# iKrishneel/fcn_object_detector

Measured on AMD Instinct MI355X. Metric: frames/sec forward 448x448 @1 GPU; train imgs/sec @1/2/4/8 GPUs, higher is better.
Workload: dtype f32

## Files before the change

### fcn_object_detector_amd/csrc/train.hip

```cpp
#include <math.h>

#include <type_traits>

#include "common.h"

using namespace fcn;

typedef float f32x16 __attribute__((ext_vector_type(16)));
typedef float v4f __attribute__((ext_vector_type(4)));

namespace {

typedef const void __attribute__((address_space(1))) * gvoid_cptr;
typedef void __attribute__((address_space(3))) * lds_ptr;
typedef float __attribute__((address_space(1))) * gf_ptr;

template <int N>
__device__ __forceinline__ void wait_vmcnt() { asm volatile("s_waitcnt vmcnt(%0)" ::"n"(N) : "memory"); }

struct WgradP {
    const float* x;
    const float* dy;
    float* dw_part;
    float* db_part;
// ... 883 lines not shown
                                                                int H, int W, int C, int dx_cstride, int dx_coffset, int k, int stride, int pad,
                                                                int OH, int OW, int dy_cstride, int dy_coffset, int accumulate,
                                                                const float* __restrict__ relu_y, int ry_cstride, int ry_coffset, int cgroups) {
    const int cg = (int)blockIdx.x % cgroups, tx = (int)blockIdx.x / cgroups;
    const int c = cg * 32 + ((int)threadIdx.x & 7) * 4;
    const int pp = (int)threadIdx.x >> 3;
    const int iy = (int)blockIdx.y * 8 + (pp >> 3), ix = tx * 8 + (pp & 7), n = (int)blockIdx.z;
    if (c >= C || iy >= H || ix >= W) return;
    const int oy_lo = max(0, (iy + pad - k + stride) / stride), oy_hi = min(OH - 1, (iy + pad) / stride);
    const int ox_lo = max(0, (ix + pad - k + stride) / stride), ox_hi = min(OW - 1, (ix + pad) / stride);
    const int me = iy * W + ix;
    v4f g = {0.f, 0.f, 0.f, 0.f};
    for (int oy = oy_lo; oy <= oy_hi; ++oy)
        for (int ox = ox_lo; ox <= ox_hi; ++ox) {
            const size_t o = ((size_t)(n * OH + oy) * OW + ox);
            const int4 id = *reinterpret_cast<const int4*>(idx + o * C + c);
            const v4f d = *reinterpret_cast<const v4f*>(dy + o * dy_cstride + dy_coffset + c);
            g[0] += id.x == me ? d[0] : 0.f;
            g[1] += id.y == me ? d[1] : 0.f;
            g[2] += id.z == me ? d[2] : 0.f;
            g[3] += id.w == me ? d[3] : 0.f;
        }
    const size_t pix = (size_t)(n * H + iy) * W + ix;
    v4f* dst = reinterpret_cast<v4f*>(dx + pix * dx_cstride + dx_coffset + c);
    if (accumulate) g += *dst;
    if (relu_y) {
        const v4f y = *reinterpret_cast<const v4f*>(relu_y + pix * ry_cstride + ry_coffset + c);
#pragma unroll
        for (int e = 0; e < 4; ++e) g[e] = y[e] > 0.f ? g[e] : 0.f;
    }
    *dst = g;
}

__global__ __launch_bounds__(256) void lrn_bwd_kernel(const float* __restrict__ x, const float* __restrict__ y, const float* __restrict__ scale,
                                                      const float* __restrict__ dy, float* __restrict__ dx, long long pixels, int C,
                                                      int x_cstride, int y_cstride, int local_size, float ratio2ab, float beta, int accumulate) {
    const long long total = pixels * C;
    const int pre = (local_size - 1) / 2;
    for (long long t = (long long)blockIdx.x * blockDim.x + threadIdx.x; t < total; t += (long long)gridDim.x * blockDim.x) {
        const int c = (int)(t % C);
        const long long pix = t / C;
        const float* yp = y + (size_t)pix * y_cstride;
        const float* dyp = dy + (size_t)pix * y_cstride;
        const float* sp = scale + (size_t)pix * C;
        float acc = 0.f;
        for (int j = c - (local_size - 1 - pre); j <= c + pre; ++j)
            if (j >= 0 && j < C) acc += dyp[j] * yp[j] / sp[j];
        const float g = dyp[c] * powf(sp[c], -beta) - ratio2ab * x[(size_t)pix * x_cstride + c] * acc;
        float* d = dx + (size_t)pix * x_cstride + c;
        *d = accumulate ? *d + g : g;
    }
}

__global__ __launch_bounds__(256) void lrn5_bwd_kernel(const float* __restrict__ x, const float* __restrict__ y, const float* __restrict__ scale,
                                                       const float* __restrict__ dy, float* __restrict__ dx, long long pixels, int C,
                                                       int x_cstride, int y_cstride, float ratio2ab, float beta, int accumulate) {
    const int cg = C / 4;
    const long long total = pixels * cg;
    const v4f zero = {0.f, 0.f, 0.f, 0.f};
    for (long long t = (long long)blockIdx.x * blockDim.x + threadIdx.x; t < total; t += (long long)gridDim.x * blockDim.x) {
        const long long pix = t / cg;
        const int g = (int)(t - pix * cg);
        const float* yp = y + (size_t)pix * y_cstride + g * 4;
        const float* dyp = dy + (size_t)pix * y_cstride + g * 4;
        const float* sp = scale + (size_t)pix * C + g * 4;
        const bool hl = g > 0, hr = g + 1 < cg;
// ... 642 lines not shown
}

int fcn_relu_bwd_f32(const float* dy, const float* y, float* dx, int pixels, int C, int cstride, fcn_stream_t s) {
    FCN_REQUIRE(dy && y && dx && pixels > 0 && C > 0 && cstride >= C, FCN_E_ARG, "relu_bwd: bad args");
    hipStream_t st = as_stream(s);
    if (cstride == C)
        hipLaunchKernelGGL(relu_bwd_kernel, dim3(stream_grid((long long)pixels * C, 256)), dim3(256), 0, st, dy, y, dx, (size_t)pixels * C);
    else
        hipLaunchKernelGGL(relu_bwd_view_kernel, dim3(stream_grid((long long)pixels * C, 256)), dim3(256), 0, st, dy, y, dx, (long long)pixels, C,
                           cstride);
    FCN_LAUNCH_CHECK("relu_bwd");
    return 0;
}

int fcn_sigmoid_bwd_f32(const float* y, const float* dy, float* dx, size_t count, int accumulate, fcn_stream_t s) {
    FCN_REQUIRE(y && dy && dx, FCN_E_ARG, "sigmoid_bwd: null");
    if (!count) return 0;
    hipLaunchKernelGGL(sigmoid_bwd_kernel, dim3(stream_grid((long long)count, 256)), dim3(256), 0, as_stream(s), y, dy, dx, count, accumulate);
    FCN_LAUNCH_CHECK("sigmoid_bwd");
    return 0;
}

int fcn_maxpool_bwd_mask_f32(const float* dy, const int32_t* idx, float* dx, int N, int H, int W, int C, int dx_cstride, int dx_coffset, int k,
                             int stride, int pad, int OH, int OW, int dy_cstride, int dy_coffset, int accumulate, const float* relu_y,
                             int relu_y_cstride, int relu_y_coffset, fcn_stream_t s) {
    FCN_REQUIRE(dy && idx && dx && N > 0 && H > 0 && W > 0 && C > 0 && k > 0 && stride > 0 && OH > 0 && OW > 0, FCN_E_ARG, "maxpool_bwd: bad args");
    FCN_REQUIRE(dx_cstride >= dx_coffset + C && dy_cstride >= dy_coffset + C, FCN_E_ARG, "maxpool_bwd: channel slice out of range");
    FCN_REQUIRE(!relu_y || (relu_y_coffset >= 0 && relu_y_cstride >= relu_y_coffset + C), FCN_E_ARG, "maxpool_bwd: mask slice out of range");
    const bool v4 = C % 4 == 0 && dx_cstride % 4 == 0 && dx_coffset % 4 == 0 && dy_cstride % 4 == 0 && dy_coffset % 4 == 0 &&
                    (long long)N * H * W * (C / 4) < (1ll << 31) && (((uintptr_t)dy | (uintptr_t)idx | (uintptr_t)dx) & 15) == 0 &&
                    (!relu_y || (relu_y_cstride % 4 == 0 && relu_y_coffset % 4 == 0 && ((uintptr_t)relu_y & 15) == 0));
    const int cgroups = (C + 31) / 32;
    const long long gx = (long long)cgroups * ((W + 7) / 8);
    if (v4 && gx < (1ll << 31) && (H + 7) / 8 <= 65535 && N <= 65535)
        hipLaunchKernelGGL(maxpool_bwd_patch_kernel, dim3((unsigned)gx, (H + 7) / 8, N), dim3(512), 0, as_stream(s), dy, idx, dx, H, W, C, dx_cstride,
                           dx_coffset, k, stride, pad, OH, OW, dy_cstride, dy_coffset, accumulate, relu_y, relu_y_cstride, relu_y_coffset, cgroups);
    else if (v4)
        hipLaunchKernelGGL(maxpool_bwd_v4_kernel, dim3(stream_grid((long long)N * H * W * (C / 4), 256)), dim3(256), 0, as_stream(s), dy, idx, dx, N, H,
                           W, C, dx_cstride, dx_coffset, k, stride, pad, OH, OW, dy_cstride, dy_coffset, accumulate, relu_y, relu_y_cstride,
                           relu_y_coffset);
    else
        hipLaunchKernelGGL(maxpool_bwd_kernel, dim3(stream_grid((long long)N * H * W * C, 256)), dim3(256), 0, as_stream(s), dy, idx, dx, N, H, W, C,
                           dx_cstride, dx_coffset, k, stride, pad, OH, OW, dy_cstride, dy_coffset, accumulate, relu_y, relu_y_cstride, relu_y_coffset);
    FCN_LAUNCH_CHECK("maxpool_bwd");
    return 0;
}

int fcn_maxpool_bwd_f32(const float* dy, const int32_t* idx, float* dx, int N, int H, int W, int C, int dx_cstride, int dx_coffset, int k,
                        int stride, int pad, int OH, int OW, int dy_cstride, int dy_coffset, int accumulate, fcn_stream_t s) {
    return fcn_maxpool_bwd_mask_f32(dy, idx, dx, N, H, W, C, dx_cstride, dx_coffset, k, stride, pad, OH, OW, dy_cstride, dy_coffset, accumulate,
                                    nullptr, 0, 0, s);
}

int fcn_deconv_depthwise_bwd_f32(const float* dy, const float* w, float* dx, int N, int H, int W, int C, int dx_cstride, int k, int stride,
                                 int pad, int OH, int OW, int dy_cstride, int dy_coffset, int accumulate, fcn_stream_t s) {
    FCN_REQUIRE(dy && w && dx && N > 0 && H > 0 && W > 0 && C > 0 && k > 0 && stride > 0 && pad >= 0, FCN_E_ARG, "deconv_bwd: bad args");
    FCN_REQUIRE(OH == stride * (H - 1) + k - 2 * pad && OW == stride * (W - 1) + k - 2 * pad, FCN_E_ARG,
                "deconv_bwd: OH/OW do not match s(H-1)+k-2p");
    FCN_REQUIRE(dx_cstride >= C && dy_coffset >= 0 && dy_cstride >= dy_coffset + C, FCN_E_ARG, "deconv_bwd: channel slice out of range");
    hipLaunchKernelGGL(deconv_dw_bwd_kernel, dim3(stream_grid((long long)N * H * W * C, 256)), dim3(256), 0, as_stream(s), dy, w, dx, N, H, W, C,
                       dx_cstride, k, stride, pad, OH, OW, dy_cstride, dy_coffset, accumulate);
    FCN_LAUNCH_CHECK("deconv_depthwise_bwd");
    return 0;
}

size_t fcn_softmax_loss_workspace_bytes(void) { return (size_t)SML_MAX_BLOCKS * 2 * sizeof(double) + 64; }

int fcn_softmax_loss_f32(const float* x, const float* label, float* dx, float* d_loss, int N, int pixels, int C, int x_cstride,
                         int label_cstride, int normalize, int has_ignore, int ignore_label, float weight, void* d_workspace, fcn_stream_t s) {
    FCN_REQUIRE(x && label && d_loss && d_workspace && N > 0 && pixels > 0 && C > 0 && x_cstride >= C && label_cstride >= 1, FCN_E_ARG,
                "softmax_loss: bad args");
    FCN_REQUIRE(((uintptr_t)d_workspace & 7) == 0, FCN_E_ALIGN, "softmax_loss: workspace must be 8-byte aligned");
    hipStream_t st = as_stream(s);
    int blocks = cdiv(pixels, 256);
    if (blocks > SML_MAX_BLOCKS) blocks = SML_MAX_BLOCKS;
    double* partial = reinterpret_cast<double*>(d_workspace);
    float* d_scale = reinterpret_cast<float*>(partial + (size_t)SML_MAX_BLOCKS * 2);
    hipLaunchKernelGGL(softmax_loss_partial_kernel, dim3(blocks), dim3(256), 0, st, x, label, dx, partial, (long long)pixels, C, x_cstride,
                       label_cstride, has_ignore, ignore_label);
    hipLaunchKernelGGL(softmax_loss_final_kernel, dim3(1), dim3(64), 0, st, partial, blocks, d_loss, d_scale, N, normalize, weight);
    if (dx) hipLaunchKernelGGL(scale_view_kernel, dim3(stream_grid((long long)pixels * C, 256)), dim3(256), 0, st, dx, d_scale, (long long)pixels, C,
                               x_cstride);
    FCN_LAUNCH_CHECK("softmax_loss");
    return 0;
// ... 62 lines not shown
```

### fcn_object_detector_amd/lib.py

```python
from __future__ import annotations

import ctypes as C
import os
import threading
from typing import Optional

_HERE = os.path.dirname(os.path.abspath(__file__))
LIB_PATH = os.environ.get("FCN_LIB_PATH") or os.path.join(_HERE, "libfcnhip.so")


class FcnLibraryError(RuntimeError):
    pass


class FcnError(RuntimeError):
    def __init__(self, code: int, msg: str):
        super().__init__("libfcnhip error %d: %s" % (code, msg))
        self.code = code


class ConvDesc(C.Structure):
    _fields_ = [
        ("x", C.c_void_p), ("w", C.c_void_p), ("bias", C.c_void_p), ("y", C.c_void_p), ("y2", C.c_void_p),
        ("N", C.c_int32), ("H", C.c_int32), ("W", C.c_int32), ("Cin", C.c_int32), ("x_cstride", C.c_int32),
# ... 11 lines not shown
class ConvGroup(C.Structure):
    _fields_ = [("d_probs", C.c_void_p), ("n", C.c_int32), ("cfg", C.c_int32), ("total_tiles", C.c_int32)]


class SolverSeg(C.Structure):
    _fields_ = [("offset", C.c_uint64), ("count", C.c_uint64), ("lr_mult", C.c_float), ("decay_mult", C.c_float)]


class LayoutDesc(C.Structure):
    _fields_ = [("src", C.c_void_p), ("dst", C.c_void_p)] + [(k, C.c_int32) for k in ("N", "C", "H", "W", "src_cstride", "src_coffset")]


class PoolDesc(C.Structure):
    _fields_ = [("x", C.c_void_p), ("y", C.c_void_p), ("idx", C.c_void_p)] + [(k, C.c_int32) for k in (
        "N", "H", "W", "C", "x_cstride", "k", "stride", "pad", "OH", "OW", "y_cstride", "y_coffset", "f16")]


class SceneObj(C.Structure):
    _fields_ = [("img", C.c_void_p), ("mask", C.c_void_p)] + [(k, C.c_int32) for k in (
        "src_h", "src_w", "flip", "roi_x", "roi_y", "roi_w", "roi_h", "out_w", "out_h", "cx", "cy", "label1")]


class ColorParams(C.Structure):
    _fields_ = [("sharpen_centre", C.c_float), ("sharpen_off", C.c_float), ("add", C.c_int32 * 3), ("mul", C.c_float * 3),
                ("gray_alpha", C.c_float), ("gray_keep", C.c_float)]


GAUSS_MAX_RADIUS = 15


class FlipSeg(C.Structure):
    _fields_ = [("w_offset", C.c_uint64), ("wt_offset", C.c_uint64), ("Cout", C.c_int32), ("kh", C.c_int32), ("kw", C.c_int32),
                ("Cin", C.c_int32), ("Cin4", C.c_int32), ("Cout4", C.c_int32)]


class DetectParams(C.Structure):
    _fields_ = [
        ("num_classes", C.c_int32), ("gy", C.c_int32), ("gx", C.c_int32), ("cell_w", C.c_int32), ("cell_h", C.c_int32),
        ("cvg_cstride", C.c_int32), ("cvg_coffset", C.c_int32), ("box_cstride", C.c_int32), ("box_coffset", C.c_int32),
        ("prob_thresh", C.c_float), ("group_thresh", C.c_int32), ("eps", C.c_double), ("min_height", C.c_int32),
        ("round_mode", C.c_int32), ("max_out", C.c_int32),
    ]


CONV_RELU, CONV_SIGMOID2, CONV_ACCUM, CONV_OUT_F32, CONV_F16, CONV_OUT_F16, CONV_MASK = 1, 2, 4, 8, 16, 32, 64
CONV_IMAGE_ONES = 128
ELT_PROD, ELT_SUM, ELT_MAX = 0, 1, 2
RECT_ROUND_NEAREST_EVEN, RECT_ROUND_TRUNCATE = 0, 1

_vp, _i, _f, _d, _sz = C.c_void_p, C.c_int, C.c_float, C.c_double, C.c_size_t

PROTOTYPES = {
    "fcn_abi_version": (_i, []),
    "fcn_last_error_string": (C.c_char_p, []),
    "fcn_device_count": (_i, [C.POINTER(_i)]),
    "fcn_init": (_i, [_i]),
    "fcn_device_name": (_i, [C.c_char_p, _i]),
    "fcn_device_sync": (_i, []),
    "fcn_malloc": (_i, [C.POINTER(_vp), _sz]),
    "fcn_free": (_i, [_vp]),
    "fcn_host_malloc": (_i, [C.POINTER(_vp), _sz]),
    "fcn_host_free": (_i, [_vp]),
    "fcn_memset_async": (_i, [_vp, _i, _sz, _vp]),
    "fcn_memcpy_h2d_async": (_i, [_vp, _vp, _sz, _vp]),
    "fcn_memcpy_d2h_async": (_i, [_vp, _vp, _sz, _vp]),
    "fcn_memcpy_d2d_async": (_i, [_vp, _vp, _sz, _vp]),
# ... 54 lines not shown
    "fcn_conv2d_wgrad_workspace_floats_cfg": (_sz, [C.POINTER(ConvDesc), _i, C.POINTER(_i)]),
    "fcn_conv2d_wgrad_cfg_f32": (_i, [C.POINTER(ConvDesc), _vp, _vp, _vp, _i, _vp]),
    "fcn_conv2d_wgrad_group_workspace_floats_cfg": (_sz, [C.POINTER(ConvDesc), _i, _i]),
    "fcn_conv2d_wgrad_group_cfg_f32": (_i, [C.POINTER(ConvDesc), _vp, _vp, _i, _vp, _i, _vp]),
    "fcn_conv_weights_flip_f32": (_i, [_vp, _vp, _i, _i, _i, _i, _i, _i, _vp]),
    "fcn_nchw_f32_to_nhwc_f16": (_i, [_vp, _vp, _i, _i, _i, _i, _i, _i, _f, _vp]),
    "fcn_nhwc_f16_to_nchw_f32": (_i, [_vp, _vp, _i, _i, _i, _i, _i, _i, _vp]),
    "fcn_maxpool_fwd_f16": (_i, [_vp, _vp] + [_i] * 12 + [_vp]),
    "fcn_lrn_fwd_f16": (_i, [_vp, _vp, _i, _i, _i, _i, _i, _f, _f, _f, _vp]),
    "fcn_avepool_fwd_f16": (_i, [_vp, _vp] + [_i] * 12 + [_vp]),
    "fcn_deconv_depthwise_fwd_f16": (_i, [_vp, _vp, _vp, _vp] + [_i] * 13 + [_vp]),
    "fcn_eltwise_fwd_f16": (_i, [_vp, _vp, _vp, _sz, _i, _f, _f, _vp]),
    "fcn_softmax_fwd_f16": (_i, [_vp, _vp, _i, _i, _i, _i, _i, _vp]),
    "fcn_copy_channels_f16": (_i, [_vp, _vp, _i, _i, _i, _i, _i, _i, _vp]),
    "fcn_preprocess_bgr8_batch": (_i, [_vp, _i, _i, _i, _vp, _i, _i, _i, _i, _f, _vp, _vp]),
    "fcn_preprocess_bgr8_rois": (_i, [_vp, _i, _i, _vp, _i, _vp, _i, _i, _i, _i, _f, _vp, _vp]),
    "fcn_preprocess_bgr8_f16": (_i, [_vp, _i, _i, _vp, _i, _i, _i, _f, _vp, _vp]),
    "fcn_compose_scene_bgr8": (_i, [_vp, _i, _i, _i, _i, _i, _i, _vp, _i, _i, _vp, _vp, _i, _i, _vp]),
    "fcn_mask_to_label_f32": (_i, [_vp, _i, _i, _vp, _i, _i, _i, _vp]),
    "fcn_compose_scene_view_bgr8": (_i, [_vp, _i, _i, _i, _i, _i, _i, _vp, _i, _i, _vp, _vp, _i, _i, _i, _i, _i, _i, _vp]),
    "fcn_blur_gauss_bgr8": (_i, [_vp, _vp, _vp, _i, _i, _vp, _i, _vp]),
    "fcn_blur_box_bgr8": (_i, [_vp, _vp, _i, _i, _i, _vp]),
    "fcn_blur_median_bgr8": (_i, [_vp, _vp, _i, _i, _i, _vp]),
    "fcn_color_augment_bgr8": (_i, [_vp, _vp, _i, _i, _vp, _vp]),
    "fcn_softmax_fwd_f32": (_i, [_vp, _vp, _i, _i, _i, _i, _vp]),
    "fcn_softmax_loss_workspace_bytes": (_sz, []),
    "fcn_softmax_loss_f32": (_i, [_vp, _vp, _vp, _vp, _i, _i, _i, _i, _i, _i, _i, _i, _f, _vp, _vp]),
    "fcn_deconv_depthwise_bwd_f32": (_i, [_vp, _vp, _vp] + [_i] * 13 + [_vp]),
    "fcn_conv_weights_flip_batch_f32": (_i, [_vp, _vp, _vp, _i, _vp]),
    "fcn_relu_bwd_f32": (_i, [_vp, _vp, _vp, _i, _i, _i, _vp]),
    "fcn_sigmoid_bwd_f32": (_i, [_vp, _vp, _vp, _sz, _i, _vp]),
    "fcn_maxpool_bwd_f32": (_i, [_vp, _vp, _vp] + [_i] * 14 + [_vp]),
    "fcn_maxpool_bwd_mask_f32": (_i, [_vp, _vp, _vp] + [_i] * 14 + [_vp, _i, _i, _vp]),
    "fcn_lrn_bwd_f32": (_i, [_vp, _vp, _vp, _vp, _vp, _i, _i, _i, _i, _i, _f, _f, _i, _vp]),
    "fcn_dropout_f32": (_i, [_vp, _vp] + [_i] * 8 + [_f, C.c_uint, C.c_uint, _vp]),
    "fcn_stream_wait_event": (_i, [_vp, _vp]),
    "fcn_comm_unique_id": (_i, [C.c_char_p]),
    "fcn_comm_init": (_i, [C.POINTER(_vp), C.c_char_p, _i, _i]),
    "fcn_comm_allreduce_sum_f32": (_i, [_vp, _vp, _sz, _vp]),
    "fcn_comm_destroy": (_i, [_vp]),
    "fcn_loss_f32": (_i, [_i, _vp, _vp, _vp, _vp, _i, _i, _i, _i, _f, _vp]),
    "fcn_sgd_update_f32": (_i, [_vp, _vp, _vp, _vp, _i, _f, _f, _f, _f, _vp]),
    "fcn_adam_update_f32": (_i, [_vp, _vp, _vp, _vp, _vp, _i, _f, _f, _f, _f, _f, _i, _f, _vp]),
}

HW_QUEUES: dict = {}
_lib: Optional[C.CDLL] = None
_lock = threading.Lock()


def load() -> C.CDLL:
    global _lib
    if _lib is not None:
        return _lib
    with _lock:
        if _lib is not None:
            return _lib
        if not os.path.isfile(LIB_PATH):
            raise FcnLibraryError(
                "libfcnhip.so not found at %s — build it with `python -c 'import __graft_entry__ as g; g.build()'` "
                "or `make -C fcn_object_detector_amd/csrc`. There is no CPU fallback." % LIB_PATH)
        global HW_QUEUES
        if "GPU_MAX_HW_QUEUES" in os.environ:
            HW_QUEUES = {"value": os.environ["GPU_MAX_HW_QUEUES"], "set_by": "environment"}
        elif os.environ.get("FCN_SET_HW_QUEUES", "1") != "0":
            os.environ["GPU_MAX_HW_QUEUES"] = "16"
# ... 33 lines not shown
```

### fcn_object_detector_amd/train.py

```python
from __future__ import annotations

import ctypes as C
import os
import math
from typing import Callable, Dict, List, Optional, Sequence, Tuple

import numpy as np

from . import lib as L
from . import proto
from .engine import Blob, DevView, DeviceBuffer, Engine, Op, PinnedArray, _r4
from .netspec import DATA_TYPES, LOSS_TYPES, Layer, NetSpec, kernel_stride_pad

F32 = np.float32


class SolverParams:

    def __init__(self, msg: Optional[proto.Msg] = None, **kw):
        g = (lambda k, d=None: msg.get(k, d)) if msg is not None else (lambda k, d=None: d)
        self.net = g("net", g("train_net"))
        self.base_lr = float(kw.get("base_lr", g("base_lr", 0.01)))
        self.momentum = float(kw.get("momentum", g("momentum", 0.0)))
        self.momentum2 = float(kw.get("momentum2", g("momentum2", 0.999)))
# ... 184 lines not shown

        def emit_dgrads(name: str, items: List[Tuple[L.ConvDesc, float]], targets: List[str]) -> dict:
            rec = dict(name=name, descs=[it[0] for it in items], targets=list(targets), grp=L.ConvGroup())
            rec["op"] = Op("dgrad", name, lambda st, g=rec["grp"]: L.check(lib.fcn_conv2d_fwd_group_f32(C.byref(g), st)), sum(it[1] for it in items))
            ops.append(rec["op"])
            dgrad_records.append(rec)
            return rec

        def finish_dgrads() -> None:
            for x, rop in relu_ops.items():
                w = writers.get(x, [])
                rec = w[-1] if w else None
                if not isinstance(rec, dict) or rop not in ops:
                    continue
                if "pool" in rec:
                    if rec["pool"] == x:
                        rec["mask"] = (B[x].buf.ptr, B[x].cstride, B[x].coffset)
                        ops.remove(rop)
                    continue
                d = rec["descs"][rec["targets"].index(x)]
                act = B[x]
                d.y2, d.y2_cstride, d.y2_coffset = act.buf.ptr, act.cstride, act.coffset
                d.flags |= L.CONV_MASK
                ops.remove(rop)
            for rec in dgrad_records:
                n_ = len(rec["descs"])
                arr = (L.ConvDesc * n_)(*rec["descs"])
                gws = DeviceBuffer(int(lib.fcn_conv2d_group_workspace_bytes(n_)), zero=False)
                cfg = self._tuned_cfg("dgrad:" + rec["name"], arr, n_, gws) if self.autotune else -1
                L.call("fcn_conv2d_group_prepare", arr, n_, gws.ptr, cfg, C.byref(rec["grp"]))
                self._keep.extend([arr, gws, rec["grp"]])
                self._group_workspaces.append(gws)
                rec["op"].name = "%s [cfg%d %dwg]" % (rec["name"], rec["grp"].cfg, rec["grp"].total_tiles)

        def wgrad_item(l: Layer, gtop: Blob):
            xb, yb = B[l.bottoms[0]], B[l.tops[0]]
            k, s, pad = kernel_stride_pad(l.sub("convolution_param"))
            n, cin, h, w = xb.shape
            _, cout, oh, ow = yb.shape
            if gtop.coffset % 4 or gtop.cstride % 4:
                raise NotImplementedError("gradient view of %s is not 16-byte aligned" % l.tops[0])
            d = L.ConvDesc()
            d.x, d.y = xb.ptr, gtop.buf.ptr
            d.N, d.H, d.W, d.Cin, d.x_cstride = n, h, w, _r4(cin), xb.cstride
            d.Cout, d.kh, d.kw, d.pad, d.stride, d.OH, d.OW = cout, k, k, pad, s, oh, ow
            d.y_cstride, d.y_coffset = gtop.cstride, gtop.coffset
            self._keep.append(d)
            dw = self._grad_view(l.name, 0)
            db = self._grad_view(l.name, 1) if len(self.params_dev[l.name]) > 1 else None
            return d, dw, db, 2.0 * n * cout * oh * ow * cin * k * k

        def emit_wgrads(layers_: List[Layer], gtops: List[Blob]) -> None:
            nonlocal ws_floats
            todo = [(l_, g_) for l_, g_ in zip(layers_, gtops) if self._learns(l_) and l_.name not in wgrad_done]
            for base in range(0, len(todo), 4):
                chunk = todo[base:base + 4]
                its = [wgrad_item(l_, g_) for l_, g_ in chunk]
                names = [l_.name for l_, _ in chunk]
                sel = {"cfg": -1}
                cfgs = [-1] + (list(range(int(lib.fcn_conv2d_wgrad_num_configs()))) if self.autotune else [])
                if len(its) == 1:
                    d, dw, db, fl = its[0]
                    ws_floats = max([ws_floats] + [int(lib.fcn_conv2d_wgrad_workspace_floats_cfg(C.byref(d), c, None)) for c in cfgs])
                    op = Op("wgrad", names[0], lambda st, d=d, dw=dw, db=db, sel=sel: L.check(lib.fcn_conv2d_wgrad_cfg_f32(
                        C.byref(d), dw.ptr, db.ptr if db else None, self._ws.ptr, sel["cfg"], st)), fl)
                else:
# ... 113 lines not shown
                for bn in l.bottoms:
                    gb = G.get(bn)
                    if gb is None:
                        continue
                    if state(gb) == "full":
                        if gtop.coffset or gb.coffset or gb.cstride != gtop.cstride:
                            raise NotImplementedError("Eltwise SUM backward accumulating into a channel slice")
                        ops.append(Op("eltwise_bwd", l.name + ":" + bn, lambda st, a=gtop, b=gb: L.check(lib.fcn_eltwise_fwd_f32(
                            a.ptr, b.ptr, b.ptr, a.pixels * a.cstride, L.ELT_SUM, 1.0, 1.0, st))))
                    else:
                        ops.append(Op("eltwise_bwd", l.name + ":" + bn, lambda st, a=gtop, b=gb: L.check(lib.fcn_copy_channels_f32(
                            a.buf.ptr, b.buf.ptr, a.pixels, a.channels, a.cstride, a.coffset, b.cstride, b.coffset, st))))
                    mark(gb)
                continue
            gbot = G.get(l.bottoms[0]) if l.bottoms else None
            if gbot is None:
                continue
            acc = 1 if state(gbot) == "full" else 0
            pool_writer = None
            if t == "Pooling":
                pp = l.sub("pooling_param")
                if str(pp.get("pool", "MAX")) != "MAX":
                    raise NotImplementedError("backward of AVE pooling (%s)" % l.name)
                xb, yb = B[l.bottoms[0]], B[l.tops[0]]
                n, c, h, w = xb.shape
                _, _, oh, ow = yb.shape
                k, s, pad = kernel_stride_pad(pp)
                idx = self.aux_dev[l.name]
                prec = dict(pool=l.bottoms[0], mask=(None, 0, 0))
                ops.append(Op("maxpool_bwd", l.name, lambda st, a=gtop, b=gbot, idx=idx, g=(n, h, w, c), kk=(k, s, pad, oh, ow), acc=acc, r=prec:
                              L.check(lib.fcn_maxpool_bwd_mask_f32(a.buf.ptr, idx.ptr, b.buf.ptr, g[0], g[1], g[2], g[3], b.cstride, b.coffset,
                                                                   kk[0], kk[1], kk[2], kk[3], kk[4], a.cstride, a.coffset, acc, r["mask"][0],
                                                                   r["mask"][1], r["mask"][2], st))))
                pool_writer = prec
            elif t == "LRN":
                xb, yb = B[l.bottoms[0]], B[l.tops[0]]
                p = l.sub("lrn_param")
                ls, al, be = int(p.get("local_size", 5)), float(p.get("alpha", 1.0)), float(p.get("beta", 0.75))
                sc = self.aux_dev[l.name]
                if gtop.coffset or gbot.coffset or xb.coffset or yb.coffset:
                    raise NotImplementedError("LRN backward on channel slices")
                ops.append(Op("lrn_bwd", l.name, lambda st, x=xb, y=yb, sc=sc, a=gtop, b=gbot, q=(ls, al, be), acc=acc: L.check(
                    lib.fcn_lrn_bwd_f32(x.ptr, y.ptr, sc.ptr, a.ptr, b.ptr, x.pixels, x.channels, x.cstride, y.cstride, q[0], q[1], q[2], acc, st))))
            elif t == "Dropout":
                if acc:
                    raise NotImplementedError("dropout backward into an already written gradient")
                ratio = float(l.sub("dropout_param").get("dropout_ratio", 0.5))
                n, c, h, w = B[l.bottoms[0]].shape
                ops.append(Op("dropout_bwd", l.name, lambda st, a=gtop, b=gbot, g=(n, c, h, w), r=ratio: L.check(lib.fcn_dropout_f32(
                    a.buf.ptr, b.buf.ptr, g[0], g[1], g[2], g[3], a.cstride, a.coffset, b.cstride, b.coffset, r, self.dropout_seed,
                    self.dropout_index_offset, st))))
            elif t == "Eltwise":
                p = l.sub("eltwise_param")
                opname = str(p.get("operation", "SUM"))
                if opname != "PROD" or len(l.bottoms) != 2:
                    raise NotImplementedError("backward of Eltwise %s" % l.name)
                if l.bottoms[1] in self.need_grad:
                    raise NotImplementedError("Eltwise PROD backward w.r.t. both bottoms (%s)" % l.name)
                if acc:
                    raise NotImplementedError("Eltwise backward into an already written gradient")
                other = B[l.bottoms[1]]
                count = gtop.pixels * gtop.cstride
                if gtop.coffset or gbot.coffset or other.coffset or other.cstride != gtop.cstride:
                    raise NotImplementedError("Eltwise backward on channel slices")
                ops.append(Op("eltwise_bwd", l.name, lambda st, a=gtop, o=other, b=gbot, n=count: L.check(lib.fcn_eltwise_fwd_f32(
                    a.ptr, o.ptr, b.ptr, n, L.ELT_PROD, 1.0, 1.0, st))))
            elif t == "Deconvolution":
                if any(m != 0.0 for m in l.lr_mult) or not l.lr_mult:
                    raise NotImplementedError("learnable Deconvolution %s (the reference freezes its bilinear upsampling, lr_mult 0)" % l.name)
                p = l.sub("convolution_param")
                k, s, pad = kernel_stride_pad(p)
                xb, yb = B[l.bottoms[0]], B[l.tops[0]]
                n, c, h, w = xb.shape
                _, _, oh, ow = yb.shape
                wdev = self.params_dev[l.name][0].ptr
                ops.append(Op("deconv_bwd", l.name, lambda st, a=gtop, b=gbot, g=(n, h, w, c, k, s, pad, oh, ow), acc=acc, wdev=wdev: L.check(
                    lib.fcn_deconv_depthwise_bwd_f32(a.buf.ptr, wdev, b.ptr, g[0], g[1], g[2], g[3], b.cstride, g[4], g[5], g[6], g[7], g[8],
                                                     a.cstride, a.coffset, acc, st))))
            elif t == "Sigmoid":
                yb = B[l.tops[0]]
                ops.append(Op("sigmoid_bwd", l.name, lambda st, y=yb, a=gtop, b=gbot, acc=acc: L.check(
                    lib.fcn_sigmoid_bwd_f32(y.ptr, a.ptr, b.ptr, y.pixels * y.cstride, acc, st))))
            elif t == "ReLU":
                yb = B[l.tops[0]]
                ops.append(Op("relu_bwd", l.name, lambda st, y=yb, a=gtop, b=gbot: L.check(lib.fcn_relu_bwd_f32(
                    a.ptr, y.ptr, b.ptr, y.pixels, y.channels, y.cstride, st))))
            elif t == "Power":
                continue
            else:
                raise NotImplementedError("backward of layer type %s (%s)" % (t, l.name))
            mark(gbot, pool_writer)
        finish_dgrads()
        self._ws = DeviceBuffer(ws_floats * 4, zero=False)
        self.bwd_ops = ops
        if self.autotune:
            self._tune_wgrads()
        self._plan_buckets()

    def _tune_wgrads(self) -> None:
        lib = L.load()
        ncfg = int(lib.fcn_conv2d_wgrad_num_configs())
        cache = self._load_tune_cache()
        e0, e1 = C.c_void_p(), C.c_void_p()
        L.call("fcn_event_create", C.byref(e0))
        L.call("fcn_event_create", C.byref(e1))
        dirty = False
        for op in self.bwd_ops:
            if op.kind != "wgrad":
                continue
            key = self._tune_key("wgrad:" + "+".join(op.layers))
            if self._tune_from is not None and key in self._tune_from._chosen_cfgs:
                op.sel["cfg"] = self._chosen_cfgs[key] = self._tune_from._chosen_cfgs[key]
                continue
            if cache is not None and key in cache and 0 <= int(cache[key]) < ncfg:
                op.sel["cfg"] = self._chosen_cfgs[key] = int(cache[key])
                continue
            best, best_ms = -1, 1e30
            timed = []
            for cfg in range(ncfg):
                op.sel["cfg"] = cfg
                for _ in range(2):
                    op.run(self.stream)
                L.call("fcn_event_record", e0, self.stream)
                for _ in range(5):
                    op.run(self.stream)
# ... 206 lines not shown
                    L.call("fcn_event_record", e0, self.comm_stream)
                for b in self.buckets:
                    self.comm.all_reduce_sum(scratch.ptr + 4 * b["offset"], b["count"], self.comm_stream)
            L.call("fcn_event_record", e1, self.comm_stream)
            L.call("fcn_event_sync", e1)
            ms = C.c_float()
            L.call("fcn_event_elapsed_ms", e0, e1, C.byref(ms))
            L.call("fcn_event_destroy", e0)
            L.call("fcn_event_destroy", e1)
            scratch.free()
        nbytes = 4 * sum(b["count"] for b in self.buckets)
        us = ms.value * 1e3 / reps
        g = self.comm.world
        return {"allreduce_us": us, "bytes": nbytes, "buckets": len(self.buckets),
                "bus_GBps": (2.0 * (g - 1) / g * nbytes / (us * 1e-6) / 1e9) if us > 0 else 0.0}

    def step_end(self) -> Dict[str, float]:
        with self.lock:
            L.call("fcn_event_sync", self._step_done)
            for b in self.blobs.values():
                b.host_valid = b.is_input
            for nm in self._in_flight:
                self.blobs[nm].host_valid = False
            out = {k: float(v[0]) for k, v in self.loss_host.items()}
            out["total_loss"] = float(sum(self.loss_blobs[k] * out[k] for k in self.loss_blobs))
            out.setdefault("loss", out["total_loss"])
            self.iter += 1
            return out

    DYNAMIC_KINDS = ("dropout", "dropout_bwd")

    def _wgrad_stream(self) -> Optional[int]:
        import os
        if os.environ.get("FCN_WGRAD_STREAM", "1") == "0":
            return None
        if getattr(self, "_side_stream", None) is None:
            sp, ev = C.c_void_p(), C.c_void_p()
            L.call("fcn_stream_create", C.byref(sp))
            L.call("fcn_event_create", C.byref(ev))
            self._side_stream, self._side_done = int(sp.value), ev
        return self._side_stream

    def _step_plan(self) -> List[Tuple[str, object]]:
        if getattr(self, "_plan", None) is not None:
            return self._plan
        import os
        first = not getattr(self, "_warm", False)
        self._warm = True
        use_graph = os.environ.get("FCN_TRAIN_GRAPH", "1") != "0" and os.environ.get("FCN_NO_GRAPH", "0") in ("", "0") and not first
        triggers: Dict[int, List[dict]] = {}
        for b in self.buckets:
            triggers.setdefault(b["after_op"], []).append(b)
        seq: List[Tuple[str, object]] = [("op", op) for op in self.ops]
        for i, op in enumerate(self.bwd_ops):
            seq.append(("op", op))
            if i in triggers:
                seq.append(("reduce", triggers[i]))
        plan: List[Tuple[str, object]] = []
        run: List[Op] = []

        def flush() -> None:
            if not run:
                return
            if use_graph and len(run) > 1:
                L.call("fcn_graph_begin", self.stream)
                try:
                    for op in run:
# ... 137 lines not shown
```

### include/fcnhip.h

```cpp
#ifndef FCNHIP_H_
#define FCNHIP_H_

#include <stddef.h>
#include <stdint.h>

#ifdef __cplusplus
extern "C" {
#endif

#define FCN_ABI_VERSION 1

#define FCN_E_ARG       1
#define FCN_E_ALIGN     2
#define FCN_E_UNSUPPORTED 3
#define FCN_E_STATE     4
#define FCN_E_CAPACITY  5

typedef void* fcn_stream_t;
typedef void* fcn_event_t;
typedef void* fcn_graph_t;
typedef void* fcn_comm_t;

int  fcn_abi_version(void);
const char* fcn_last_error_string(void);
// ... 205 lines not shown
                     uint8_t* pmap, int frame_h, int frame_w, void* d_workspace, int32_t* out, fcn_stream_t s);

int  fcn_gen_targets(const int32_t* rects, const int32_t* labels, const int32_t* rect_offsets, int batch,
                     int num_classes, int gy, int gx, int stride, double iou_thresh,
                     float* foreground, float* bbox, float* size, float* obj, float* cvg_block,
                     fcn_stream_t s);
int  fcn_gen_targets_nhwc(const int32_t* rects, const int32_t* labels, const int32_t* rect_offsets, int batch,
                          int num_classes, int gy, int gx, int stride, double iou_thresh,
                          float* foreground, int fg_cstride, float* bbox, float* size, float* obj, float* cvg_block,
                          int blk_cstride, fcn_stream_t s);

size_t fcn_conv2d_wgrad_workspace_floats(const fcn_conv_desc* h_d, int* h_splits);
int  fcn_conv2d_wgrad_f32(const fcn_conv_desc* h_d, float* dw, float* db, float* d_workspace, fcn_stream_t s);
size_t fcn_conv2d_wgrad_group_workspace_floats(const fcn_conv_desc* h_ds, int n);
int  fcn_conv2d_wgrad_group_f32(const fcn_conv_desc* h_ds, float* const* h_dws, float* const* h_dbs, int n, float* d_workspace,
                                fcn_stream_t s);
int  fcn_conv2d_wgrad_num_configs(void);
int  fcn_conv2d_wgrad_split_config(void);
size_t fcn_conv2d_wgrad_workspace_floats_cfg(const fcn_conv_desc* h_d, int cfg_request, int* h_splits);
int  fcn_conv2d_wgrad_cfg_f32(const fcn_conv_desc* h_d, float* dw, float* db, float* d_workspace, int cfg_request, fcn_stream_t s);
size_t fcn_conv2d_wgrad_group_workspace_floats_cfg(const fcn_conv_desc* h_ds, int n, int cfg_request);
int  fcn_conv2d_wgrad_group_cfg_f32(const fcn_conv_desc* h_ds, float* const* h_dws, float* const* h_dbs, int n, float* d_workspace,
                                    int cfg_request, fcn_stream_t s);
int  fcn_conv_weights_flip_f32(const float* w, float* wt, int Cout, int kh, int kw, int Cin, int Cin4, int Cout4, fcn_stream_t s);
typedef struct fcn_flip_seg { uint64_t w_offset, wt_offset; int32_t Cout, kh, kw, Cin, Cin4, Cout4; } fcn_flip_seg;
int  fcn_conv_weights_flip_batch_f32(const float* w_base, float* wt_base, const fcn_flip_seg* d_segs, int nseg, fcn_stream_t s);
int  fcn_relu_bwd_f32(const float* dy, const float* y, float* dx, int pixels, int C, int cstride, fcn_stream_t s);
int  fcn_sigmoid_bwd_f32(const float* y, const float* dy, float* dx, size_t count, int accumulate, fcn_stream_t s);
int  fcn_maxpool_bwd_f32(const float* dy, const int32_t* idx, float* dx, int N, int H, int W, int C, int dx_cstride, int dx_coffset,
                         int k, int stride, int pad, int OH, int OW, int dy_cstride, int dy_coffset, int accumulate, fcn_stream_t s);
int  fcn_maxpool_bwd_mask_f32(const float* dy, const int32_t* idx, float* dx, int N, int H, int W, int C, int dx_cstride, int dx_coffset,
                              int k, int stride, int pad, int OH, int OW, int dy_cstride, int dy_coffset, int accumulate,
                              const float* relu_y, int relu_y_cstride, int relu_y_coffset, fcn_stream_t s);
int  fcn_lrn_bwd_f32(const float* x, const float* y, const float* scale, const float* dy, float* dx, int pixels, int C,
                     int x_cstride, int y_cstride, int local_size, float alpha, float beta, int accumulate, fcn_stream_t s);
int  fcn_dropout_f32(const float* x, float* y, int N, int C, int H, int W, int x_cstride, int x_coffset, int y_cstride,
                     int y_coffset, float ratio, unsigned seed, unsigned index_offset, fcn_stream_t s);
int  fcn_loss_f32(int kind, const float* a, const float* b, float* da, float* d_loss, int pixels, int C, int cstride, int num,
                  float weight, fcn_stream_t s);
size_t fcn_softmax_loss_workspace_bytes(void);
int  fcn_softmax_loss_f32(const float* x, const float* label, float* dx, float* d_loss, int N, int pixels, int C, int x_cstride,
                          int label_cstride, int normalize, int has_ignore, int ignore_label, float weight, void* d_workspace,
                          fcn_stream_t s);
int  fcn_deconv_depthwise_bwd_f32(const float* dy, const float* w, float* dx, int N, int H, int W, int C, int dx_cstride, int k,
                                  int stride, int pad, int OH, int OW, int dy_cstride, int dy_coffset, int accumulate, fcn_stream_t s);
typedef struct fcn_solver_seg { uint64_t offset, count; float lr_mult, decay_mult; } fcn_solver_seg;
int  fcn_sgd_update_f32(float* w, const float* g, float* hist, const fcn_solver_seg* d_segs, int nseg, float rate, float momentum,
                        float weight_decay, float grad_scale, fcn_stream_t s);
int  fcn_adam_update_f32(float* w, const float* g, float* m, float* v, const fcn_solver_seg* d_segs, int nseg, float rate,
                         float beta1, float beta2, float delta, float weight_decay, int t, float grad_scale, fcn_stream_t s);

int  fcn_comm_unique_id(char* h_id128);
int  fcn_comm_init(fcn_comm_t* comm, const char* h_id128, int world, int rank);
int  fcn_comm_allreduce_sum_f32(fcn_comm_t comm, float* buf, size_t count, fcn_stream_t s);
int  fcn_comm_destroy(fcn_comm_t comm);

#ifdef __cplusplus
}
#endif
#endif
```

Measured before the change: 3551.

## Add LDS-tiled grouped maxpool backward for 3x3 stride-1 pools

Adds a new maxpool backward kernel for 3x3 stride-1 pad-1 pools. It stages a 10x10 halo of dy and argmax indices in LDS per 8x8 tile and 32-channel group, then gathers from shared memory instead of issuing repeated global loads. A grouped launch batches up to four independent pool-backward ops into one kernel, with per-problem parameters read from kernarg, to cut launch count; the training graph builder merges consecutive non-aliasing pool ops. It also makes the side wgrad stream default depend on the reported hardware queue count.

Measured after the change: 3544 (median of 6 runs). About the same (-0.2%).

```diff
diff --git a/fcn_object_detector_amd/csrc/train.hip b/fcn_object_detector_amd/csrc/train.hip
--- a/fcn_object_detector_amd/csrc/train.hip
+++ b/fcn_object_detector_amd/csrc/train.hip
@@ -939,6 +939,99 @@
     *dst = g;
 }
 
+constexpr int kMaxPoolGroup = 4;
+struct PoolBwdP {
+    const float* dy;
+    const int32_t* idx;
+    float* dx;
+    const float* relu_y;
+    int H, W, C, dx_cstride, dx_coffset, dy_cstride, dy_coffset, ry_cstride, ry_coffset, accumulate, cgroups, tiles_x, tiles_y, pad_;
+};
+struct PoolBwdGroupArgs {
+    int n;
+    int blk_end[kMaxPoolGroup];
+    PoolBwdP p[kMaxPoolGroup];
+};
+
+__global__ __launch_bounds__(512) void maxpool_bwd_lds_kernel(const PoolBwdGroupArgs a) {
+    __shared__ v4f s_dy[100 * 8];
+    typedef int v4i __attribute__((ext_vector_type(4)));
+    __shared__ v4i s_id[100 * 8];
+    const int b = blockIdx.x;
+    int pi = 0, begin = 0;
+#pragma unroll
+    for (int i = 0; i < kMaxPoolGroup - 1; ++i) {
+        const bool past = i + 1 < a.n && b >= a.blk_end[i];
+        pi += past ? 1 : 0;
+        begin = past ? a.blk_end[i] : begin;
+    }
+    typedef const PoolBwdGroupArgs __attribute__((address_space(4))) * karg_ptr;
+    karg_ptr ka = (karg_ptr)__builtin_amdgcn_kernarg_segment_ptr();
+    union { PoolBwdP p; unsigned w[sizeof(PoolBwdP) / 4]; } u;
+    const unsigned __attribute__((address_space(4)))* src = (const unsigned __attribute__((address_space(4)))*)&ka->p[pi];
+#pragma unroll
+    for (int i = 0; i < (int)(sizeof(PoolBwdP) / 4); ++i) u.w[i] = src[i];
+    const PoolBwdP& p = u.p;
+    typedef const v4f __attribute__((address_space(1))) * gv4_cptr;
+    typedef const v4i __attribute__((address_space(1))) * gi4_cptr;
+    typedef v4f __attribute__((address_space(1))) * gv4_ptr;
+    int t = b - begin;
+    const int cg = t % p.cgroups;
+    t /= p.cgroups;
+    const int tx = t % p.tiles_x;
+    t /= p.tiles_x;
+    const int ty = t % p.tiles_y, n = t / p.tiles_y;
+    const int q = (int)threadIdx.x & 7, c = cg * 32 + q * 4;
+    const bool c_ok = c < p.C;
+    const v4i none = {-1, -1, -1, -1};
+    const v4f zero = {0.f, 0.f, 0.f, 0.f};
+#pragma unroll
+    for (int r = 0; r < 2; ++r) {
+        const int hp = ((int)threadIdx.x >> 3) + r * 64;
+        if (hp < 100) {
+            const int hy = hp / 10, oy = ty * 8 - 1 + hy, ox = tx * 8 - 1 + (hp - hy * 10);
+            v4i id = none;
+            v4f d = zero;
+            if (c_ok && (unsigned)oy < (unsigned)p.H && (unsigned)ox < (unsigned)p.W) {
+                const size_t o = (size_t)(n * p.H + oy) * p.W + ox;
+                id = *(gi4_cptr)(p.idx + o * p.C + c);
+                d = *(gv4_cptr)(p.dy + o * p.dy_cstride + p.dy_coffset + c);
+            }
+            s_id[hp * 8 + q] = id;
+            s_dy[hp * 8 + q] = d;
+        }
+    }
+    const int pp = (int)threadIdx.x >> 3, ly = pp >> 3, lx = pp & 7;
+    const int iy = ty * 8 + ly, ix = tx * 8 + lx;
+    const bool live = c_ok && iy < p.H && ix < p.W;
+    const size_t pix = (size_t)(n * p.H + iy) * p.W + ix;
+    v4f old = zero, y = zero;
+    if (live && p.accumulate) old = *(gv4_cptr)(p.dx + pix * p.dx_cstride + p.dx_coffset + c);
+    if (live && p.relu_y) y = *(gv4_cptr)(p.relu_y + pix * p.ry_cstride + p.ry_coffset + c);
+    __syncthreads();
+    if (!live) return;
+    const int me = iy * p.W + ix;
+    v4f g = zero;
+#pragma unroll
+    for (int wy = 0; wy < 3; ++wy)
+#pragma unroll
+        for (int wx = 0; wx < 3; ++wx) {
+            const int h = ((ly + wy) * 10 + lx + wx) * 8 + q;
+            const v4i id = s_id[h];
+            const v4f d = s_dy[h];
+            g[0] += id[0] == me ? d[0] : 0.f;
+            g[1] += id[1] == me ? d[1] : 0.f;
+            g[2] += id[2] == me ? d[2] : 0.f;
+            g[3] += id[3] == me ? d[3] : 0.f;
+        }
+    if (p.accumulate) g += old;
+    if (p.relu_y) {
+#pragma unroll
+        for (int e = 0; e < 4; ++e) g[e] = y[e] > 0.f ? g[e] : 0.f;
+    }
+    *(gv4_ptr)(p.dx + pix * p.dx_cstride + p.dx_coffset + c) = g;
+}
+
 __global__ __launch_bounds__(256) void lrn_bwd_kernel(const float* __restrict__ x, const float* __restrict__ y, const float* __restrict__ scale,
                                                       const float* __restrict__ dy, float* __restrict__ dx, long long pixels, int C,
                                                       int x_cstride, int y_cstride, int local_size, float ratio2ab, float beta, int accumulate) {
@@ -1647,6 +1740,13 @@
                     (!relu_y || (relu_y_cstride % 4 == 0 && relu_y_coffset % 4 == 0 && ((uintptr_t)relu_y & 15) == 0));
     const int cgroups = (C + 31) / 32;
     const long long gx = (long long)cgroups * ((W + 7) / 8);
+    const char* lds = getenv("FCN_POOL_BWD_LDS");
+    if (v4 && k == 3 && stride == 1 && pad == 1 && OH == H && OW == W && dx_coffset >= 0 && dy_coffset >= 0 && !(lds && lds[0] == '0') &&
+        (long long)N * H * W < (1ll << 31) && gx * ((H + 7) / 8) * N < (1ll << 31)) {
+        const fcn_pool_bwd_desc d = {dy, idx, dx, relu_y, N, H, W, C, dx_cstride, dx_coffset, dy_cstride, dy_coffset, relu_y ? relu_y_cstride : 0,
+                                     relu_y ? relu_y_coffset : 0, accumulate, 0};
+        return fcn_maxpool_bwd_group_f32(&d, 1, s);
+    }
     if (v4 && gx < (1ll << 31) && (H + 7) / 8 <= 65535 && N <= 65535)
         hipLaunchKernelGGL(maxpool_bwd_patch_kernel, dim3((unsigned)gx, (H + 7) / 8, N), dim3(512), 0, as_stream(s), dy, idx, dx, H, W, C, dx_cstride,
                            dx_coffset, k, stride, pad, OH, OW, dy_cstride, dy_coffset, accumulate, relu_y, relu_y_cstride, relu_y_coffset, cgroups);
@@ -1665,6 +1765,38 @@
                         int stride, int pad, int OH, int OW, int dy_cstride, int dy_coffset, int accumulate, fcn_stream_t s) {
     return fcn_maxpool_bwd_mask_f32(dy, idx, dx, N, H, W, C, dx_cstride, dx_coffset, k, stride, pad, OH, OW, dy_cstride, dy_coffset, accumulate,
                                     nullptr, 0, 0, s);
+}
+
+int fcn_maxpool_bwd_group_f32(const fcn_pool_bwd_desc* ds, int n, fcn_stream_t s) {
+    FCN_REQUIRE(ds && n > 0 && n <= kMaxPoolGroup, FCN_E_ARG, "maxpool_bwd group: need 1..%d problems", kMaxPoolGroup);
+    PoolBwdGroupArgs a;
+    memset(&a, 0, sizeof(a));
+    a.n = n;
+    long long blocks = 0;
+    for (int i = 0; i < n; ++i) {
+        const fcn_pool_bwd_desc& d = ds[i];
+        FCN_REQUIRE(d.dy && d.idx && d.dx && d.N > 0 && d.H > 0 && d.W > 0 && d.C > 0, FCN_E_ARG, "maxpool_bwd group: bad args (problem %d)", i);
+        FCN_REQUIRE(d.dx_coffset >= 0 && d.dy_coffset >= 0 && d.dx_cstride >= d.dx_coffset + d.C && d.dy_cstride >= d.dy_coffset + d.C, FCN_E_ARG,
+                    "maxpool_bwd group: channel slice out of range (problem %d)", i);
+        FCN_REQUIRE(!d.relu_y || (d.relu_y_coffset >= 0 && d.relu_y_cstride >= d.relu_y_coffset + d.C), FCN_E_ARG,
+                    "maxpool_bwd group: mask slice out of range (problem %d)", i);
+        FCN_REQUIRE(d.C % 4 == 0 && d.dx_cstride % 4 == 0 && d.dx_coffset % 4 == 0 && d.dy_cstride % 4 == 0 && d.dy_coffset % 4 == 0 &&
+                        (((uintptr_t)d.dy | (uintptr_t)d.idx | (uintptr_t)d.dx) & 15) == 0 &&
+                        (!d.relu_y || (d.relu_y_cstride % 4 == 0 && d.relu_y_coffset % 4 == 0 && ((uintptr_t)d.relu_y & 15) == 0)),
+                    FCN_E_ALIGN, "maxpool_bwd group: channels, strides, offsets and pointers must be 16-byte multiples (problem %d)", i);
+        PoolBwdP& p = a.p[i];
+        p.dy = d.dy, p.idx = d.idx, p.dx = d.dx, p.relu_y = d.relu_y;
+        p.H = d.H, p.W = d.W, p.C = d.C, p.dx_cstride = d.dx_cstride, p.dx_coffset = d.dx_coffset, p.dy_cstride = d.dy_cstride;
+        p.dy_coffset = d.dy_coffset, p.ry_cstride = d.relu_y_cstride, p.ry_coffset = d.relu_y_coffset, p.accumulate = d.accumulate;
+        p.cgroups = (d.C + 31) / 32, p.tiles_x = (d.W + 7) / 8, p.tiles_y = (d.H + 7) / 8;
+        blocks += (long long)p.cgroups * p.tiles_x * p.tiles_y * d.N;
+        FCN_REQUIRE((long long)d.N * d.H * d.W < (1ll << 31) && blocks < (1ll << 31), FCN_E_UNSUPPORTED, "maxpool_bwd group: too many workgroups");
+        a.blk_end[i] = (int)blocks;
+    }
+    for (int i = n; i < kMaxPoolGroup; ++i) a.blk_end[i] = (int)blocks;
+    hipLaunchKernelGGL(maxpool_bwd_lds_kernel, dim3((unsigned)blocks), dim3(512), 0, as_stream(s), a);
+    FCN_LAUNCH_CHECK("maxpool_bwd group");
+    return 0;
 }
 
 int fcn_deconv_depthwise_bwd_f32(const float* dy, const float* w, float* dx, int N, int H, int W, int C, int dx_cstride, int k, int stride,
diff --git a/fcn_object_detector_amd/lib.py b/fcn_object_detector_amd/lib.py
--- a/fcn_object_detector_amd/lib.py
+++ b/fcn_object_detector_amd/lib.py
@@ -67,6 +67,15 @@
 class FlipSeg(C.Structure):
     _fields_ = [("w_offset", C.c_uint64), ("wt_offset", C.c_uint64), ("Cout", C.c_int32), ("kh", C.c_int32), ("kw", C.c_int32),
                 ("Cin", C.c_int32), ("Cin4", C.c_int32), ("Cout4", C.c_int32)]
+
+
+MAX_POOL_GROUP = 4
+
+
+class PoolBwdDesc(C.Structure):
+    _fields_ = [("dy", C.c_void_p), ("idx", C.c_void_p), ("dx", C.c_void_p), ("relu_y", C.c_void_p)] + [
+        (f, C.c_int32) for f in ("N", "H", "W", "C", "dx_cstride", "dx_coffset", "dy_cstride", "dy_coffset", "relu_y_cstride",
+                                 "relu_y_coffset", "accumulate", "reserved")]
 
 
 class DetectParams(C.Structure):
@@ -187,6 +196,7 @@
     "fcn_sigmoid_bwd_f32": (_i, [_vp, _vp, _vp, _sz, _i, _vp]),
     "fcn_maxpool_bwd_f32": (_i, [_vp, _vp, _vp] + [_i] * 14 + [_vp]),
     "fcn_maxpool_bwd_mask_f32": (_i, [_vp, _vp, _vp] + [_i] * 14 + [_vp, _i, _i, _vp]),
+    "fcn_maxpool_bwd_group_f32": (_i, [_vp, _i, _vp]),
     "fcn_lrn_bwd_f32": (_i, [_vp, _vp, _vp, _vp, _vp, _i, _i, _i, _i, _i, _f, _f, _i, _vp]),
     "fcn_dropout_f32": (_i, [_vp, _vp] + [_i] * 8 + [_f, C.c_uint, C.c_uint, _vp]),
     "fcn_stream_wait_event": (_i, [_vp, _vp]),
diff --git a/fcn_object_detector_amd/train.py b/fcn_object_detector_amd/train.py
--- a/fcn_object_detector_amd/train.py
+++ b/fcn_object_detector_amd/train.py
@@ -240,6 +240,40 @@
                 self._keep.extend([arr, gws, rec["grp"]])
                 self._group_workspaces.append(gws)
                 rec["op"].name = "%s [cfg%d %dwg]" % (rec["name"], rec["grp"].cfg, rec["grp"].total_tiles)
+
+        def group_pools() -> None:
+            if os.environ.get("FCN_POOL_BWD_LDS", "1") == "0":
+                return
+            i = 0
+            while i < len(ops):
+                run: List[Op] = []
+                bufs: set = set()
+                while i + len(run) < len(ops) and len(run) < L.MAX_POOL_GROUP:
+                    op = ops[i + len(run)]
+                    pl = getattr(op, "pool", None)
+                    if pl is None:
+                        break
+                    mine = {pl["dy"].buf.ptr, pl["dx"].buf.ptr, pl["rec"]["mask"][0]} - {None}
+                    if bufs & mine:
+                        break
+                    bufs |= mine
+                    run.append(op)
+                if not run:
+                    i += 1
+                    continue
+                arr = (L.PoolBwdDesc * len(run))()
+                for d, op in zip(arr, run):
+                    pl = op.pool
+                    d.dy, d.idx, d.dx, d.relu_y = pl["dy"].buf.ptr, pl["idx"].ptr, pl["dx"].buf.ptr, pl["rec"]["mask"][0]
+                    d.N, d.H, d.W, d.C = pl["g"]
+                    d.dx_cstride, d.dx_coffset, d.dy_cstride, d.dy_coffset = pl["dx"].cstride, pl["dx"].coffset, pl["dy"].cstride, pl["dy"].coffset
+                    d.relu_y_cstride, d.relu_y_coffset, d.accumulate = pl["rec"]["mask"][1], pl["rec"]["mask"][2], pl["acc"]
+                self._keep.append(arr)
+                gop = Op("maxpool_bwd", "+".join(op.name for op in run), lambda st, arr=arr, m=len(run): L.check(
+                    lib.fcn_maxpool_bwd_group_f32(arr, m, st)))
+                gop.members = run
+                ops[i:i + len(run)] = [gop]
+                i += 1
 
         def wgrad_item(l: Layer, gtop: Blob):
             xb, yb = B[l.bottoms[0]], B[l.tops[0]]
@@ -419,6 +453,8 @@
                               L.check(lib.fcn_maxpool_bwd_mask_f32(a.buf.ptr, idx.ptr, b.buf.ptr, g[0], g[1], g[2], g[3], b.cstride, b.coffset,
                                                                    kk[0], kk[1], kk[2], kk[3], kk[4], a.cstride, a.coffset, acc, r["mask"][0],
                                                                    r["mask"][1], r["mask"][2], st))))
+                if (k, s, pad, oh, ow) == (3, 1, 1, h, w) and not (c % 4 or gtop.cstride % 4 or gtop.coffset % 4 or gbot.cstride % 4 or gbot.coffset % 4):
+                    ops[-1].pool = dict(dy=gtop, dx=gbot, idx=idx, g=(n, h, w, c), acc=acc, rec=prec)
                 pool_writer = prec
             elif t == "LRN":
                 xb, yb = B[l.bottoms[0]], B[l.tops[0]]
@@ -478,6 +514,7 @@
                 raise NotImplementedError("backward of layer type %s (%s)" % (t, l.name))
             mark(gbot, pool_writer)
         finish_dgrads()
+        group_pools()
         self._ws = DeviceBuffer(ws_floats * 4, zero=False)
         self.bwd_ops = ops
         if self.autotune:
@@ -750,7 +787,11 @@
 
     def _wgrad_stream(self) -> Optional[int]:
         import os
-        if os.environ.get("FCN_WGRAD_STREAM", "1") == "0":
+        want = os.environ.get("FCN_WGRAD_STREAM", "")
+        if want not in ("0", "1"):
+            queues = str(L.HW_QUEUES.get("value") or "")
+            want = "0" if queues.isdigit() and int(queues) <= 2 else "1"
+        if want == "0":
             return None
         if getattr(self, "_side_stream", None) is None:
             sp, ev = C.c_void_p(), C.c_void_p()
diff --git a/include/fcnhip.h b/include/fcnhip.h
--- a/include/fcnhip.h
+++ b/include/fcnhip.h
@@ -261,6 +261,12 @@
 int  fcn_maxpool_bwd_mask_f32(const float* dy, const int32_t* idx, float* dx, int N, int H, int W, int C, int dx_cstride, int dx_coffset,
                               int k, int stride, int pad, int OH, int OW, int dy_cstride, int dy_coffset, int accumulate,
                               const float* relu_y, int relu_y_cstride, int relu_y_coffset, fcn_stream_t s);
+#define FCN_MAX_POOL_GROUP 4
+typedef struct fcn_pool_bwd_desc {
+    const float* dy; const int32_t* idx; float* dx; const float* relu_y;
+    int32_t N, H, W, C, dx_cstride, dx_coffset, dy_cstride, dy_coffset, relu_y_cstride, relu_y_coffset, accumulate, reserved;
+} fcn_pool_bwd_desc;
+int  fcn_maxpool_bwd_group_f32(const fcn_pool_bwd_desc* h_ds, int n, fcn_stream_t s);
 int  fcn_lrn_bwd_f32(const float* x, const float* y, const float* scale, const float* dy, float* dx, int pixels, int C,
                      int x_cstride, int y_cstride, int local_size, float alpha, float beta, int accumulate, fcn_stream_t s);
 int  fcn_dropout_f32(const float* x, float* y, int N, int C, int H, int W, int x_cstride, int x_coffset, int y_cstride,
```
